# pmelchior/scarlet

Hardware: AMD Instinct MI355X
Metric: PGM iters/sec over batched blends; achieved HBM GB/s vs roofline (higher is better)
Workload: dtype f32; 1 GPU; configs[2]: 1024 independent 5-band 128x128 blends in total, 10 ExtendedSource components (41x41) each, ConvolutionRenderer FFT 160x160; iterations 0..1234 of a fit from the initial parameters; loop=blend, blends_total=1024, components_per_blend=10, sub_ranges_per_gpu=3

## Files before the change

### include/scarlet_amd.h

```cpp
#ifndef SCARLET_AMD_H
#define SCARLET_AMD_H

#include <stdint.h>

#ifdef __cplusplus
extern "C" {
#endif

typedef enum smi_status {
    SMI_OK = 0,
    SMI_ERR_INVALID = -1,
    SMI_ERR_HIP = -2,
    SMI_ERR_NO_DEVICE = -3,
    SMI_ERR_ARITHMETIC = -4
} smi_status;

const char *smi_last_error(void);
int smi_device_count(void);
const char *smi_version(void);


int smi_prox_weighted_monotonic_f32(float *flat_img, const float *weights,
                                    const int32_t *offsets, int32_t n_off,
                                    const int32_t *dist_idx, int32_t n_idx,
// ... 390 lines not shown
int smi_batch_restore_state(smi_batch *b);

int smi_batch_enable_timing(smi_batch *b, int32_t on);
int smi_batch_get_timing(smi_batch *b, double *ms_per_phase, int32_t n_phases);

int smi_batch_fft_shape(smi_batch *b, int32_t *fft_h, int32_t *fft_w);

int smi_batch_resize_test(smi_batch *b, int32_t *margin, double *edge_pull);
int smi_batch_get_component_states(smi_batch *b, const int32_t *components, int32_t n,
                                   float *states);
int smi_batch_update_components(smi_batch *b, const smi_components *c, const int32_t *keep,
                                const float *states);
int smi_batch_set_states(smi_batch *b, const int32_t *state);
int smi_batch_set_iteration_base(smi_batch *b, const int32_t *base);
int smi_batch_get_progress(smi_batch *b, int32_t *state, int32_t *n_loss);
int smi_batch_set_pause_at(smi_batch *b, const int32_t *it);
int smi_batch_get_converged(smi_batch *b, int32_t *flag);
int smi_batch_set_round(smi_batch *b, const int32_t *state, const int32_t *base,
                        const int32_t *pause_at);
int smi_batch_get_round(smi_batch *b, int32_t *state, int32_t *n_loss, int32_t *converged);

int64_t smi_observation_uploads(void);

int smi_batch_conv_path_used(smi_batch *b, int32_t *path);

int smi_batch_set_frame_extents(smi_batch *b, const int32_t *h, const int32_t *w);

int smi_fft_shape_for(int32_t H, int32_t W, int32_t kernel_h, int32_t kernel_w, int32_t conv_path,
                      int32_t *Fy, int32_t *Fx);

typedef struct smi_resampler smi_resampler;
int smi_resampler_create(const float *A, const float *Pt, int32_t C, int32_t n_a, int32_t n_b,
                         int32_t Fy, int32_t Fx, smi_resampler **out);
int smi_resampler_render(smi_resampler *r, const float *model, float *out);
int smi_resampler_time(smi_resampler *r, int32_t n_rep, double *ms_per_render);
int smi_resampler_destroy(smi_resampler *r);
int smi_resampler_get_path(smi_resampler *r, int32_t *path);
int smi_resampler_set_path(smi_resampler *r, int32_t path);

int smi_gemm_plan(int32_t M, int32_t N, int32_t K, int32_t n_batch, int64_t scratch_elems,
                  int32_t plan[5]);
int smi_gemm_test(const float *A, int64_t strideA, const float *B, int64_t strideB, float *C,
                  int64_t strideC, int32_t n_batch, int32_t M, int32_t N, int32_t K,
                  int64_t scratch_elems, int32_t plan[5], int32_t *guard_ok);
int smi_resampler_adjoint(smi_resampler *r, const float *resid, float *gpad);

int smi_sqrt_rn_normal_test(const float *x, float *y, int64_t n);

int smi_update_launch_plan_test(int32_t n_items, int32_t size_class, int64_t stage_bytes,
                                int32_t cu_count, int32_t range_items, int32_t finalize_pending,
                                int32_t n_ranges, int64_t plan[8]);
int smi_update_last_fold_plan_test(int64_t plan[8]);

int smi_batch_attach_lowres(smi_batch *b, smi_resampler *r, const int32_t *channels,
                            const float *data, const float *weights, double log_norm);
int smi_batch_get_lowres_rendered(smi_batch *b, int32_t index, float *out);


int smi_starlet_transform_f32(const float *d_images, int32_t n, int32_t H, int32_t W,
                              int32_t scales, int32_t generation, double *d_coeffs,
                              double *d_work, void *stream);
int smi_starlet_transform_f64(const double *d_images, int32_t n, int32_t H, int32_t W,
                              int32_t scales, int32_t generation, double *d_coeffs,
                              double *d_work, void *stream);
int smi_starlet_reconstruction_f64(const double *d_coeffs, int32_t n, int32_t H, int32_t W,
                                   int32_t scales, int32_t generation, double *d_image,
                                   double *d_work, void *stream);
int smi_multiresolution_support_f64(const double *d_coeffs, int32_t n, int32_t planes,
                                    int32_t H, int32_t W, int64_t plane_stride,
                                    int64_t image_stride, const double *sigma0,
                                    const double *thresh0, double K, double epsilon,
                                    int32_t max_iter, int32_t *d_support, double *d_masked,
                                    int32_t *iterations, void *stream);
int smi_coadd_f32(const float *d_images, int32_t bands, int32_t H, int32_t W, float *d_out,
                  void *stream);
int smi_coadd_f64(const double *d_images, int32_t bands, int32_t H, int32_t W, double *d_out,
                  void *stream);

typedef struct smi_detect_task {
    int32_t bands, h, w, scales;
    int64_t image_off, coeff_off, work_off;
    double sigma0, thresh0;
} smi_detect_task;
int smi_detect_wavelets_scratch_bytes(int32_t n, int64_t *bytes);
int smi_detect_wavelets_f32(int32_t n, const smi_detect_task *tasks, const void *d_tasks, double K,
                            double epsilon, int32_t max_iter, int32_t generation,
                            const float *d_images, int64_t n_images, double *d_coeffs,
                            int64_t n_coeffs, double *d_work, int64_t n_work, double *d_masked,
                            int32_t *d_support, int32_t *d_iterations, void *d_scratch,
                            int64_t scratch_bytes, void *stream);
int smi_detect_wavelets_f64(int32_t n, const smi_detect_task *tasks, const void *d_tasks, double K,
                            double epsilon, int32_t max_iter, int32_t generation,
                            const double *d_images, int64_t n_images, double *d_coeffs,
                            int64_t n_coeffs, double *d_work, int64_t n_work, double *d_masked,
                            int32_t *d_support, int32_t *d_iterations, void *d_scratch,
                            int64_t scratch_bytes, void *stream);

int smi_get_footprints_f32(const float *image, int32_t H, int32_t W, double min_separation,
                           int32_t min_area, int32_t thresh, int32_t *counts);
int smi_get_footprints_f64(const double *image, int32_t H, int32_t W, double min_separation,
                           int32_t min_area, int32_t thresh, int32_t *counts);
int smi_footprints_fetch(int32_t *bounds, uint8_t *masks, int32_t *peak_start, int32_t *peak_yx,
                         double *peak_flux);

int smi_footprints_device_work_bytes(int32_t P, int32_t H, int32_t W, int64_t *bytes);
int smi_footprints_device_fetch_bytes(const int32_t *counts, int64_t *bytes);
// ... 51 lines not shown
```

### scarlet_amd/_lib.py

```python

import ctypes
import os

import numpy as np

_HERE = os.path.dirname(os.path.abspath(__file__))
LIB_PATH = os.environ.get("SCARLET_AMD_LIB") or os.path.join(_HERE, "libscarlet_amd.so")

PROX_MONOTONIC = 1
PROX_SYMMETRY = 2
PROX_POSITIVE = 4
PROX_CENTER_ON = 8
PROX_NORM_MAX = 16
PROX_NORM_SUM = 32
PROX_L1 = 64
PROX_L0 = 128
PROX_FIT_CENTER = 256
PROX_BG_THRESH = 512
PROX_L_RELATIVE = 1024
PROX_MONO_MASK = 2048
SCHEME_AMSGRAD, SCHEME_FISTA = 0, 1
COMPONENT_POINT_SOURCE = 1 << 16
COMPONENT_SHIFTING = 1 << 17
COMPONENT_FIXED_SED = 1 << 18
# ... 124 lines not shown
        ctypes.c_int,
        [c_f64p, ctypes.c_int32, ctypes.c_int32, c_f64p, ctypes.c_int32, c_i32p, c_i32p,
         c_i32p, c_i32p, c_f64p],
    ),
    "smi_reweight_f32": (ctypes.c_int, _REWEIGHT(c_f32p)),
    "smi_reweight_f64": (ctypes.c_int, _REWEIGHT(c_f64p)),
    "smi_lite_spectra_f32": (ctypes.c_int, _LITE_SPECTRA(c_f32p)),
    "smi_lite_spectra_f64": (ctypes.c_int, _LITE_SPECTRA(c_f64p)),
    "smi_get_valid_monotonic_pixels_f32": (
        ctypes.c_int,
        [ctypes.c_int32, ctypes.c_int32, c_f32p, ctypes.c_int32, ctypes.c_int32, c_u8p, c_u8p,
         ctypes.c_double, c_i32p, ctypes.c_double],
    ),
    "smi_get_valid_monotonic_pixels_f64": (
        ctypes.c_int,
        [ctypes.c_int32, ctypes.c_int32, c_f64p, ctypes.c_int32, ctypes.c_int32, c_u8p, c_u8p,
         ctypes.c_double, c_i32p, ctypes.c_double],
    ),
    "smi_linear_interpolate_invalid_pixels_f32": (
        ctypes.c_int,
        [c_i32p, c_i32p, ctypes.c_int32, c_u8p, c_f32p, ctypes.c_int32, ctypes.c_int32, c_u8p,
         ctypes.c_double, ctypes.c_int32, c_i32p],
    ),
    "smi_linear_interpolate_invalid_pixels_f64": (
        ctypes.c_int,
        [c_i32p, c_i32p, ctypes.c_int32, c_u8p, c_f64p, ctypes.c_int32, ctypes.c_int32, c_u8p,
         ctypes.c_double, ctypes.c_int32, c_i32p],
    ),
    "smi_resampler_create": (
        ctypes.c_int,
        [c_f32p, c_f32p, ctypes.c_int32, ctypes.c_int32, ctypes.c_int32, ctypes.c_int32,
         ctypes.c_int32, ctypes.POINTER(ctypes.c_void_p)],
    ),
    "smi_resampler_render": (ctypes.c_int, [ctypes.c_void_p, c_f32p, c_f32p]),
    "smi_resampler_time": (ctypes.c_int, [ctypes.c_void_p, ctypes.c_int32,
                                          ctypes.POINTER(ctypes.c_double)]),
    "smi_resampler_destroy": (ctypes.c_int, [ctypes.c_void_p]),
    "smi_resampler_get_path": (ctypes.c_int, [ctypes.c_void_p, ctypes.POINTER(ctypes.c_int32)]),
    "smi_resampler_set_path": (ctypes.c_int, [ctypes.c_void_p, ctypes.c_int32]),
    "smi_resampler_adjoint": (ctypes.c_int, [ctypes.c_void_p, c_f32p, c_f32p]),
    "smi_gemm_plan": (ctypes.c_int, [ctypes.c_int32] * 4 + [ctypes.c_int64, c_i32p]),
    "smi_gemm_test": (
        ctypes.c_int,
        [c_f32p, ctypes.c_int64, c_f32p, ctypes.c_int64, c_f32p, ctypes.c_int64]
        + [ctypes.c_int32] * 4 + [ctypes.c_int64, c_i32p, c_i32p],
    ),
    "smi_sqrt_rn_normal_test": (ctypes.c_int, [c_f32p, c_f32p, ctypes.c_int64]),
    "smi_update_launch_plan_test": (
        ctypes.c_int,
        [ctypes.c_int32, ctypes.c_int32, ctypes.c_int64] + [ctypes.c_int32] * 4
        + [ctypes.POINTER(ctypes.c_int64)],
    ),
    "smi_update_last_fold_plan_test": (ctypes.c_int, [ctypes.POINTER(ctypes.c_int64)]),
    "smi_batch_attach_lowres": (
        ctypes.c_int, [ctypes.c_void_p, ctypes.c_void_p, c_i32p, c_f32p, c_f32p, ctypes.c_double]
    ),
    "smi_batch_get_lowres_rendered": (ctypes.c_int, [ctypes.c_void_p, ctypes.c_int32, c_f32p]),
    "smi_batch_create": (
        ctypes.c_int,
        [ctypes.POINTER(BatchDesc), ctypes.c_int, ctypes.POINTER(ctypes.c_void_p)],
    ),
    "smi_batch_destroy": (ctypes.c_int, [ctypes.c_void_p]),
    "smi_batch_add_sweep_plan": (
        ctypes.c_int,
        [ctypes.c_void_p, ctypes.c_int32, ctypes.c_int32, c_f64p, c_i32p, c_i32p,
         ctypes.c_int32],
    ),
    "smi_sweep_ring_plan": (
        ctypes.c_int,
        [ctypes.c_int32, ctypes.c_int32, c_f64p, c_i32p, c_i32p, ctypes.c_int32, c_i32p, c_f32p,
         ctypes.POINTER(ctypes.c_uint16), ctypes.c_int64],
    ),
    "smi_batch_set_observation": (ctypes.c_int, [ctypes.c_void_p, c_f32p, c_f32p]),
    "smi_batch_set_observation_device": (
        ctypes.c_int, [ctypes.c_void_p, ctypes.c_void_p, ctypes.c_void_p]
    ),
    "smi_batch_set_kernel": (ctypes.c_int, [ctypes.c_void_p, c_f32p]),
    "smi_batch_set_components": (ctypes.c_int, [ctypes.c_void_p, ctypes.POINTER(Components)]),
    "smi_batch_set_moments": (ctypes.c_int, [ctypes.c_void_p] + [c_f32p] * 6),
    "smi_batch_get_moments": (ctypes.c_int, [ctypes.c_void_p] + [c_f32p] * 6),
    "smi_batch_get_parameters": (ctypes.c_int, [ctypes.c_void_p, c_f32p, c_f32p]),
    "smi_batch_set_parameters": (ctypes.c_int, [ctypes.c_void_p, c_f32p, c_f32p]),
    "smi_batch_get_centers": (ctypes.c_int, [ctypes.c_void_p] + [c_f64p] * 5),
    "smi_batch_set_center_moments": (ctypes.c_int, [ctypes.c_void_p] + [c_f64p] * 3),
    "smi_batch_set_centers": (ctypes.c_int, [ctypes.c_void_p, c_f64p]),
    "smi_batch_get_model_morphology": (ctypes.c_int, [ctypes.c_void_p, c_f32p]),
    "smi_batch_get_starlet": (ctypes.c_int, [ctypes.c_void_p] + [c_f32p] * 5),
    "smi_batch_get_profiles": (ctypes.c_int, [ctypes.c_void_p] + [c_f64p] * 5),
    "smi_batch_set_profile_moments": (ctypes.c_int, [ctypes.c_void_p] + [c_f64p] * 3),
    "smi_profile_probe": (ctypes.c_int, [ctypes.c_int, ctypes.c_int32, c_f64p] + [ctypes.c_int32] * 4
                          + [c_f64p]),
    "smi_batch_set_starlet_moments": (ctypes.c_int, [ctypes.c_void_p] + [c_f32p] * 3),
    "smi_starlet_monotonic_mask_f32": (
        ctypes.c_int,
        [c_f32p, ctypes.c_int32, ctypes.c_int32, ctypes.c_int32, ctypes.c_int32, ctypes.c_double,
         ctypes.c_int32],
    ),
    "smi_batch_set_scheme": (ctypes.c_int, [ctypes.c_void_p, ctypes.c_int32]),
    "smi_batch_get_fista_state": (ctypes.c_int, [ctypes.c_void_p, c_f32p, c_f32p, c_f64p]),
    "smi_batch_set_fista_state": (ctypes.c_int, [ctypes.c_void_p, c_f32p, c_f32p, c_f64p]),
    "smi_batch_set_log_norm": (ctypes.c_int, [ctypes.c_void_p, ctypes.c_int32]),
    "smi_batch_add_observation": (ctypes.c_int, [ctypes.c_void_p, c_f32p, c_f32p, c_f32p]),
    "smi_batch_add_loss_constant": (ctypes.c_int, [ctypes.c_void_p, ctypes.POINTER(ctypes.c_double)]),
    "smi_batch_set_previous_loss": (ctypes.c_int, [ctypes.c_void_p, c_f64p]),
    "smi_batch_set_sub_ranges": (ctypes.c_int, [ctypes.c_void_p, ctypes.c_int32]),
    "smi_batch_get_sub_ranges": (ctypes.c_int, [ctypes.c_void_p, c_i32p]),
# ... 215 lines not shown
```

### scarlet_amd/csrc/batch.hip

```cpp
#include <rocfft/rocfft.h>

#include <algorithm>
#include <cmath>
#include <cstdlib>
#include <atomic>
#include <cstring>
#include <limits>
#include <map>
#include <mutex>
#include <thread>
#include <tuple>
#include <utility>

#include "common.h"

namespace smi {

static thread_local std::string g_error;
static std::atomic<int> g_hw_queues{4};
static std::atomic<long long> g_observation_uploads{0};
static std::mutex g_plan_mutex;
void set_error(const std::string &msg) { g_error = msg; }

static int next_fast_len(int n) {
// ... 615 lines not shown
                  int64_t scratch_elems, int32_t plan[5], int32_t *guard_ok) {
    SMI_REQUIRE(A && B && C && plan && guard_ok && scratch_elems >= 0, "bad argument");
    int ndev = 0;
    if (hipGetDeviceCount(&ndev) != hipSuccess || ndev == 0) {
        set_error("no HIP device available");
        return SMI_ERR_NO_DEVICE;
    }
    GemmPlan p;
    *guard_ok = 0;
    const int rc = gemm_test(A, strideA, B, strideB, C, strideC, n_batch, M, N, K,
                             (size_t)scratch_elems, &p, guard_ok);
    plan[0] = p.tm; plan[1] = p.tn; plan[2] = p.bk; plan[3] = p.kslice; plan[4] = p.n_slices;
    return rc;
}

int smi_sqrt_rn_normal_test(const float *x, float *y, int64_t n) {
    SMI_REQUIRE(x && y, "null argument");
    if (int rc = have_device()) return rc;
    return sqrt_rn_normal_test(x, y, n);
}

static void put_update_plan(const UpdateLaunchPlan &p, int64_t plan[8]) {
    plan[0] = p.pack;
    plan[1] = p.n_blocks;
    plan[2] = p.persistent;
    plan[3] = p.stage;
    plan[4] = (int64_t)p.lds;
    plan[5] = (int64_t)p.lds_table;
    plan[6] = p.gather_off;
    plan[7] = p.fold;
}

int smi_update_launch_plan_test(int32_t n_items, int32_t size_class, int64_t stage_bytes,
                                int32_t cu_count, int32_t range_items, int32_t finalize_pending,
                                int32_t n_ranges, int64_t plan[8]) {
    SMI_REQUIRE(plan, "null argument");
    SMI_REQUIRE(n_ranges >= 1 && n_items > 0 && range_items >= n_items && size_class >= 0 &&
                    size_class < kNumUpdateClasses && cu_count > 0 &&
                    stage_bytes < ((int64_t)1 << 31),
                "update_launch_plan_test: bad argument");
    const UpdateLaunchPlan p = update_launch_plan(n_items, size_class, stage_bytes, cu_count,
                                                  range_items, finalize_pending != 0, n_ranges > 1,
                                                  UpdateLaunchSwitches());
    put_update_plan(p, plan);
    return SMI_OK;
}

int smi_update_last_fold_plan_test(int64_t plan[8]) {
    SMI_REQUIRE(plan, "null argument");
    put_update_plan(update_last_fold_plan(), plan);
    return SMI_OK;
}

static constexpr int kMaxLowRes = 8;

int smi_batch_attach_lowres(smi_batch *b, smi_resampler *r, const int32_t *channels,
                            const float *data, const float *weights, double log_norm) {
    SMI_REQUIRE(b && r && channels && data && weights, "null argument");
    SMI_REQUIRE(b->d.n_blends == 1, "a low-resolution observation needs a batch of one blend");
    SMI_REQUIRE(!b->frame_hw, "a low-resolution observation does not support frame extents");
    SMI_REQUIRE(r->impl, "resampler already destroyed");
    SMI_REQUIRE((int)b->lowres.size() < kMaxLowRes, "too many low-resolution observations");
    SMI_HIP(hipSetDevice(b->device));
    SMI_HIP(hipStreamSynchronize(b->stream));
    if (!b->extra_terms) {
        SMI_HIP(dev_alloc(&b->extra_terms, kMaxLowRes));
        SMI_HIP(hipMemset(b->extra_terms, 0, kMaxLowRes * sizeof(double)));
    }
    LowRes *l = nullptr;
    int rc = lowres_create(r->impl, channels, data, weights, log_norm, b->d.H, b->d.W,
                           b->extra_terms + b->lowres.size(), &l);
    if (rc) {
        lowres_destroy(l);
        return rc;
    }
    b->lowres.push_back(l);
    refresh_view(b);
    return SMI_OK;
}

int smi_batch_get_lowres_rendered(smi_batch *b, int32_t index, float *out) {
    SMI_REQUIRE(b && out, "null argument");
    SMI_REQUIRE(index >= 0 && index < (int)b->lowres.size(), "no such low-resolution observation");
    return lowres_get_rendered(b->lowres[index], out, b->stream);
}

int smi_resampler_destroy(smi_resampler *r) {
    if (!r) return SMI_OK;
    resampler_destroy(r->impl);
    delete r;
    return SMI_OK;
}

int smi_get_valid_monotonic_pixels_f32(int32_t i, int32_t j, const float *image, int32_t rows,
                                       int32_t cols, uint8_t *unchecked, uint8_t *orphans,
                                       double variance, int32_t *bounds, double thresh) {
    return seam1_mask_valid<float>(i, j, image, rows, cols, unchecked, orphans, variance, bounds, thresh);
}
int smi_get_valid_monotonic_pixels_f64(int32_t i, int32_t j, const double *image, int32_t rows,
                                       int32_t cols, uint8_t *unchecked, uint8_t *orphans,
                                       double variance, int32_t *bounds, double thresh) {
    return seam1_mask_valid<double>(i, j, image, rows, cols, unchecked, orphans, variance, bounds, thresh);
}
int smi_linear_interpolate_invalid_pixels_f32(const int32_t *ri, const int32_t *ci, int32_t n,
                                              uint8_t *unchecked, float *model, int32_t rows,
                                              int32_t cols, uint8_t *orphans, double variance,
// ... 2300 lines not shown
```

### scarlet_amd/csrc/common.h

```cpp
#pragma once

#include <hip/hip_runtime.h>
#include <stdint.h>

#include <string>
#include <vector>

#include "../../include/scarlet_amd.h"

namespace smi {

void set_error(const std::string &msg);

#define SMI_HIP(expr)                                                              \
    do {                                                                           \
        hipError_t _e = (expr);                                                    \
        if (_e != hipSuccess) {                                                    \
            smi::set_error(std::string(#expr) + ": " + hipGetErrorString(_e));     \
            return SMI_ERR_HIP;                                                    \
        }                                                                          \
    } while (0)

#define SMI_REQUIRE(cond, msg)                                                     \
    do {                                                                           \
// ... 287 lines not shown
              GemmPlan *plan, int32_t *guard_ok);
struct LowRes;
int lowres_create(Resampler *r, const int32_t *channels, const float *data, const float *weights,
                  double log_norm, int H, int W, double *term_slot, LowRes **out);
void lowres_destroy(LowRes *l);
int lowres_evaluate(LowRes *l, const float *P, int Py, int Px, int backward, hipStream_t s);
void lowres_add_gradient(LowRes *l, float *Q, int Py, int Px, hipStream_t s);
int lowres_get_rendered(LowRes *l, float *out, hipStream_t s);
int launch_sweep_timing(const SweepPlanDev *d_plans, const SweepPlanDev &host_plan, int plan_id,
                        int mode, int n_rep, float one_minus_g, int waves, int groups,
                        long long *cycles, float *images, hipStream_t s);
int sqrt_rn_normal_test(const float *x, float *y, int64_t n);
enum UpdateFold : int32_t {
    kFoldNone = 0,
    kFoldTrailing = 1,
    kFoldInGrid = 2,
    kFoldSeparate = 3,
};
struct UpdateLaunchSwitches {
    int32_t forced_pack = 0, forced_blocks = 0;
    bool may_stage = true, may_persist = true;
    int32_t fold_mode = 2;
};
struct UpdateLaunchPlan {
    int32_t pack = 1;
    int32_t n_blocks = 0;
    int32_t persistent = 0;
    int32_t stage = 0;
    int32_t gather_off = -1;
    int32_t fold = kFoldNone;
    size_t lds = 0, lds_table = 0;
};
UpdateLaunchPlan update_last_fold_plan();
UpdateLaunchPlan update_launch_plan(int32_t n_items, int32_t cls, int64_t stage_bytes, int32_t cus,
                                    int32_t range_items, bool pending, bool shared,
                                    const UpdateLaunchSwitches &sw);
void launch_resize_test(const BatchView &v, int32_t *margin, double *pull, hipStream_t s);
void launch_gather_states(const BatchView &v, const int32_t *sel, const int64_t *off, int32_t n_sel,
                          float *staging, hipStream_t s);
void launch_scatter_states(const BatchView &v, const int64_t *off, const float *staging,
                           hipStream_t s);
void launch_carry_states(const int32_t *keep, const int64_t *old_moff, const int64_t *new_moff,
                         int32_t n, float *const from[4], float *const to[4], hipStream_t s);
void launch_interleave_obs(const float *data, const float *weights, float4 *dw, int64_t planes,
                           int32_t H, int32_t W, hipStream_t s);
void launch_log_norm(const float *weights, double *log_norm, int32_t nb, int64_t n,
                     hipStream_t s);
void launch_wrap_kernel(const float *kern, float *out, int32_t n_img, int32_t ph,
                        int32_t pw, int32_t Fy, int32_t Fx, float scale, hipStream_t s);
void launch_crop(const float *P, float *out, int32_t n_img, int32_t H, int32_t W,
                 int32_t Fy, int32_t Fx, hipStream_t s);
void launch_count_active(const int32_t *state, int32_t nb, int32_t *out, hipStream_t s);

bool fused_conv_supported(int Fy, int Fx);
bool fused_conv_instantiated(int Fy, int Fx);
bool fused_conv_choose(int ny, int nx, int *Fy, int *Fx);
int launch_fused_conv(const BatchView &v, int Fy, int Fx, const float *model, const float2 *Kt,
                      int k_bands, int k_per_blend, float *out, int mode, long long *dbg,
                      hipStream_t s);
int launch_fused_conv_short(const BatchView &v, int Fy, int Fx, const float *model,
                            const float2 *Kt, int k_bands, int k_per_blend, float *out, int mode,
                            long long *dbg, hipStream_t s);
int launch_stamp_spectrum(const float *d_kern, double2 *d_tmp, float2 *Kt, int n_img, int ph,
                          int pw, int Fy, int Fx, double scale, hipStream_t s);
int launch_permute_kernel_spectrum(const float2 *Khat, float2 *Kt, int n_img, int Fy, int Fx,
                                   float scale, hipStream_t s);

template <typename T>
int sweep_host_buffers(T *flat_img, int32_t n_pix, const SweepPlanHost &plan, T min_gradient);
template <typename T>
int sweep_many_host_buffers(T *images, int32_t n_img, int32_t n_pix,
                            const std::vector<SweepPlanHost> &plans, T min_gradient);
template <typename T>
int apply_filter_host_buffers(const T *image, int32_t H, int32_t W, const T *values,
                              int32_t n_taps, const int32_t *ys, const int32_t *ye,
                              const int32_t *xs, const int32_t *xe, T *result);

}
```

### scarlet_amd/csrc/fused_conv.hip

```cpp
#include <cstdlib>
#include <type_traits>

#include "common.h"
#include "fft_regs.h"

namespace smi {

using fftk::cf;
using fftk::cmul;
using fftk::cmulc;
using fftk::ld;
using fftk::st;

namespace {

#ifndef SMI_CONV_THREADS
#define SMI_CONV_THREADS 1024
#endif
constexpr int kThreads = SMI_CONV_THREADS;
constexpr int kF2 = 16;

constexpr int conv_column_stride(int fy) { return ((fy + fy / kF2 + 3) / 8) * 8 + 4; }
constexpr size_t conv_lds_bytes(int fy, int fx) {
    return sizeof(float2) * ((size_t)(fx / 2) * conv_column_stride(fy) + 2 * fy + fx) +
// ... 315 lines not shown
                xa[k2] = ld(z[k2 * C::SY]);
                xb[k2] = ld(z[k2 * C::SY + 1]);
            }
            __builtin_amdgcn_sched_barrier(0);
            if (trip == 0) mid();
            __builtin_amdgcn_sched_barrier(0);
            auto tail = [&] {
                fftk::Dft<kF2, true>::run(va);
#pragma unroll
                for (int i = 0; i < 8; ++i) {
                    z[i * C::SY] = st(va[2 * i]);
                    z[i * C::SY + 1] = st(va[2 * i + 1]);
                }
            };
            if (b.kind == 0) {
#pragma unroll
                for (int k2 = 0; k2 < 8; ++k2) {
                    va[k2] = plus(xa[k2], xb[k2]);
                    va[15 - k2] = from_partner(minus(xa[k2], xb[k2]));
                }
                tail();
            } else if (b.kind == 1) {
                va[0] = cf{xa[0].x, xb[0].x};
                va[8] = cf{xa[0].y, xb[0].y};
#pragma unroll
                for (int k2 = 1; k2 < 8; ++k2) {
                    va[k2] = plus(xa[k2], xb[k2]);
                    va[16 - k2] = minus(xa[k2], xb[k2]);
                }
                tail();
            } else {
#pragma unroll
                for (int k2 = 0; k2 < 8; ++k2) {
                    va[k2] = plus(xa[k2], xb[k2]);
                    va[15 - k2] = minus(xa[k2], xb[k2]);
                }
                tail();
            }
        }
        lds_barrier();
    }
};


template <int FX1, int NX1, int M>
struct ModelGather {
    static constexpr uint32_t kNone = 0x40000000u;
    const BatchView &v;
    int band_c, H, W, y, n2, ylo;
    struct Lanes {
        int oy, ox, h, w, mo;
        float sd;
    };
    __device__ __forceinline__ int open(unsigned long long &todo, const Lanes &l, float &sd,
                                        cf (&mv)[M]) const {
        const bool none = todo == 0;
        const int kl = none ? 0 : __builtin_ctzll(todo);
        todo &= todo - 1;
        const int oy = __builtin_amdgcn_readlane(l.oy, kl), hh = __builtin_amdgcn_readlane(l.h, kl);
        const int ox = __builtin_amdgcn_readlane(l.ox, kl), w = __builtin_amdgcn_readlane(l.w, kl);
        const float *mbase = v.morph + __builtin_amdgcn_readlane(l.mo, kl);
        const plane_t r = band_plane(mbase, hh * w);
        sd = __builtin_bit_cast(float, __builtin_amdgcn_readlane(__builtin_bit_cast(int, l.sd), kl));
        const int n1lo = (ox > 0 ? ox : 0) >> 4;
        const uint32_t hlim = none ? 0u : (uint32_t)min(hh, H - oy);
        const uint32_t wlim4 = 4u * (uint32_t)min(w, W - ox);
        const uint32_t ry = (uint32_t)(y - oy), w4 = 4u * (uint32_t)w;
        uint32_t row0, row1;
        asm("v_mul_u32_u24 %0, %1, %2" : "=v"(row0) : "v"(ry), "s"(w4));
        asm("v_mul_u32_u24 %0, %1, %2" : "=v"(row1) : "v"(ry + 1u), "s"(w4));
        row0 = ry < hlim ? row0 : kNone;
        row1 = ry + 1u < hlim ? row1 : kNone;
        const uint32_t x4 = (uint32_t)(16 * n1lo + n2 - ox) * 4u;
#pragma unroll
        for (int m = 0; m < M; ++m) {
            uint32_t t = x4 + 64u * m;
            t = t < wlim4 ? t : kNone;
            mv[m].x = __builtin_bit_cast(float, __builtin_amdgcn_raw_buffer_load_b32(r, row0 + t, 0, 0));
            mv[m].y = __builtin_bit_cast(float, __builtin_amdgcn_raw_buffer_load_b32(r, row1 + t, 0, 0));
        }
        return none ? -1 : n1lo;
    }
    __device__ __forceinline__ void close(int n1lo_, float sd_, const cf (&mv)[M], cf (&acc)[FX1]) const {
        const cf sd = cf{sd_, sd_};
        fftk::static_for<0, NX1>([&](auto lo) {
            constexpr int n1lo = decltype(lo)::value;
            if (n1lo_ == n1lo) {
#pragma unroll
                for (int m = 0; m < M; ++m)
                    if (n1lo + m < NX1) acc[n1lo + m] = fftk::fma2(mv[m], sd, acc[n1lo + m]);
                asm volatile("; n1lo = %0" ::"n"(n1lo));
            }
        });
    }
    __device__ __forceinline__ void run(int b, int lane, cf (&acc)[FX1]) const {
#pragma unroll
        for (int n1 = 0; n1 < NX1; ++n1) acc[n1] = cf{0.f, 0.f};
        const int cs = v.comp_start[b], ce = v.comp_start[b + 1];
        for (int kb = cs; kb < ce; kb += 64) {
            const int kk = kb + lane;
            const bool have = kk < ce;
            Lanes l;
            l.oy = have ? v.c_oy[kk] : 0;
            l.ox = have ? v.c_ox[kk] : 0;
            l.h = have ? v.c_h[kk] : 0;
            l.w = have ? v.c_w[kk] : 0;
            l.mo = have ? (int)v.c_moff[kk] : 0;
            l.sd = have ? v.sed[kk * v.C + band_c] : 0.f;
            const bool hit = have && l.oy < ylo + 8 && l.oy + l.h > ylo && l.oy < H && l.ox < W &&
                             l.ox + l.w > 0;
            unsigned long long todo = __ballot(hit);
            if (!todo) continue;
            cf mva[M], mvb[M];
            float sda, sdb;
            int na = open(todo, l, sda, mva);
            for (;;) {
                const int nb = open(todo, l, sdb, mvb);
                close(na, sda, mva, acc);
                if (nb < 0) break;
                na = open(todo, l, sda, mva);
                close(nb, sdb, mvb, acc);
                if (na < 0) break;
            }
        }
    }
};

extern __shared__ __attribute__((aligned(16))) float2 lds_conv[];

template <int FY1, int FX1, int ZB, bool EXT>
__global__ __launch_bounds__(kThreads) void fused_conv_kernel(BatchView v, const float *model,
                                                              const float2 *Kt, int k_bands,
                                                              int k_per_blend, float *out,
                                                              int mode, long long *dbg) {
    using C = Cfg<FY1, FX1, ZB>;
    constexpr int NX1 = C::NX1;
    const int total = gridDim.x;
    int lid = blockIdx.x;
    if (total % 8 == 0) lid = (blockIdx.x % 8) * (total / 8) + blockIdx.x / 8;
    const int b = lid / v.C + v.blend0, c = lid % v.C;
    if (v.state[b] >= 2) return;
    const int tid = threadIdx.x;
    const int H = v.H, W = v.W;
    const int Hb = EXT ? v.frame_h(b) : H, Wb = EXT ? v.frame_w(b) : W;

    Conv<FY1, FX1, ZB> cv;
    cv.T = lds_conv;
    cv.twy = cv.T + C::NT * C::SY;
    cv.twx = cv.twy + C::FY;
    cv.tid = tid;
    cv.n_pairs = (H + 1) / 2;
    cv.first_block_item();
    cv.qtab = cv.twx + C::FX;
    double *loss_part = reinterpret_cast<double *>(cv.qtab + C::FY);
    const int64_t band = ((int64_t)b * v.C + c) * H * W;
    const int n_items = cv.stride_items();
    using Item = typename Conv<FY1, FX1, ZB>::StrideItem;

    const bool have_cube = model != nullptr;
    const plane_t r_model = band_plane(have_cube ? model + band : v.data + band, H * W);
    cf mrow[FX1];
    auto fetch_model = [&](const Item &s) {
        const PairRows a = pair_rows(2 * s.j, s.n2, W);
        fftk::static_for<0, NX1>([&](auto n1c) {
            constexpr int n1 = decltype(n1c)::value;
            mrow[n1] = pair_load<n1>(r_model, a);
        });
    };
    auto render_rows = [&](const Item &s) {
        const int j0 = __builtin_amdgcn_readfirstlane(s.j - ((tid & 63) >> 4));
        if (v.render_slots <= 4) {
            const ModelGather<FX1, NX1, 4> g{v, c, Hb, Wb, 2 * s.j, s.n2, 2 * j0};
            g.run(b, tid & 63, mrow);
        } else {
            const ModelGather<FX1, NX1, (FX1 < 6 ? FX1 : 6)> g{v, c, Hb, Wb, 2 * s.j, s.n2, 2 * j0};
            g.run(b, tid & 63, mrow);
        }
    };
    if (have_cube) fetch_model(cv.stride_item(tid));
    for (int j = tid; j < C::FY; j += kThreads) {
        float s, co;
        sincospif(2.0f * (float)((j / kF2) * (j % kF2)) / (float)C::FY, &s, &co);
        cv.twy[j] = make_float2(co, -s);
    }
    for (int j = tid; j < C::FX; j += kThreads) {
        float s, co;
        sincospif(2.0f * (float)((j / kF2) * (j % kF2)) / (float)C::FX, &s, &co);
        cv.twx[j] = make_float2(co, -s);
    }
    {
        const int y0 = 2 * cv.n_pairs, tail = kF2 * C::NY1 - y0;
        for (int i = tid; i < tail * C::NT; i += kThreads)
            cv.T[(i / tail) * C::SY + sk(y0 + i % tail)] = make_float2(0.f, 0.f);
    }
    const float2 *K = Kt + ((int64_t)(k_per_blend ? b : 0) * k_bands + (k_bands == 1 ? 0 : c)) *
                               C::FY * C::NKX;
    for (int j = tid; j < C::FY; j += kThreads) cv.qtab[j] = K[(int64_t)(C::FX / 2) * C::FY + j];
    __syncthreads();
#ifndef SMI_DBG_BLOCK
#define SMI_DBG_BLOCK 0
#endif
#define SMI_STAMP(i) if (dbg && tid == 0 && blockIdx.x == SMI_DBG_BLOCK) dbg[i] = clock64()
    SMI_STAMP(0);

    for (int it = tid; (have_cube ? it : it - (tid & 63)) < n_items; it += kThreads) {
        const Item s = cv.stride_item(it);
        if (have_cube) {
            if (it != tid) fetch_model(s);
#pragma unroll
            for (int n1 = 0; n1 < NX1; ++n1)
                if (kF2 * n1 + s.n2 >= W) mrow[n1] = cf{0.f, 0.f};
        } else {
            render_rows(s);
        }
        if (s.on) cv.stride_forward(mrow, s);
    }
    lds_barrier();
    SMI_STAMP(6);
    cv.blocks_forward();
    SMI_STAMP(1);
    cv.columns(K, false);
    SMI_STAMP(2);
    double loss = 0.0;
    {
        cf loss2 = cf{0.f, 0.f};
        const int64_t pband = ((int64_t)b * v.C + c) * cv.n_pairs * W;
        const char *p_dw = reinterpret_cast<const char *>(v.dw + pband);
        const plane_t r_rendered = band_plane(out + band, H * W);
#ifndef SMI_CONV_PRE
#define SMI_CONV_PRE 8
#endif
        constexpr int kPre = SMI_CONV_PRE < NX1 ? SMI_CONV_PRE : NX1;
        cf dv[NX1], wv[NX1];
        auto fetch = [&](const Item &s, auto from, auto to) {
            uint32_t o = (uint32_t)(min(s.j, cv.n_pairs - 1) * W + s.n2) * 16u;
            asm volatile("" : "+v"(o));
            fftk::static_for<decltype(from)::value, decltype(to)::value>([&](auto n1c) {
                constexpr int n1 = decltype(n1c)::value;
                dw_load<n1>(p_dw, o, dv[n1], wv[n1]);
            });
        };
        using std::integral_constant;
        const Item s0 = cv.stride_item(tid);
        fetch(s0, integral_constant<int, 0>{}, integral_constant<int, kPre>{});
        constexpr int kLate = NX1 > 8 ? NX1 - 8 : 0;
        cv.blocks_inverse([&] { fetch(s0, integral_constant<int, kPre>{}, integral_constant<int, NX1 - kLate>{}); });
        SMI_STAMP(10);
        for (int it = tid; it < n_items; it += kThreads) {
            const Item s = cv.stride_item(it);
            const int y = 2 * s.j;
            if (it != tid) fetch(s, integral_constant<int, 0>{}, integral_constant<int, NX1 - kLate>{});
            cf m[FX1];
            cv.stride_inverse(m, s);
            fetch(s, integral_constant<int, NX1 - kLate>{}, integral_constant<int, NX1>{});
#pragma unroll
            for (int n1 = 0; n1 < NX1; ++n1) {
                const int x = kF2 * n1 + s.n2;
                if (mode == 1) {
                    plane_store(r_rendered, y, x, W, m[n1].x);
                    plane_store(r_rendered, y + 1, x, W, m[n1].y);
                }
                const cf w = x < W ? wv[n1] : cf{0.f, 0.f};
                const cf d = m[n1] - dv[n1];
                m[n1] = w * d;
// ... 55 lines not shown
    *kn = make_float2(0.5f * (a.x - b.x), 0.5f * (a.y - b.y));
}

__global__ void stamp_dft_x(const float *kern, double2 *A, int ph, int pw, int Fx, int NKX) {
    const int img = blockIdx.y;
    const int i = blockIdx.x * blockDim.x + threadIdx.x;
    if (i >= ph * NKX) return;
    const int dy = i / NKX, kx = i - dy * NKX;
    double re = 0.0, im = 0.0;
    for (int dx = 0; dx < pw; ++dx) {
        int t = (kx * (dx - pw / 2)) % Fx;
        if (t < 0) t += Fx;
        double s, c;
        sincospi(2.0 * (double)t / (double)Fx, &s, &c);
        const double k = (double)kern[((int64_t)img * ph + dy) * pw + dx];
        re += k * c;
        im -= k * s;
    }
    A[(int64_t)img * ph * NKX + i] = make_double2(re, im);
}

template <int FY1>
__global__ void stamp_dft_y(const double2 *A, float2 *Kt, int ph, int NKX, double scale) {
    constexpr int FY = FY1 * kF2;
    const int img = blockIdx.y;
    const int i = blockIdx.x * blockDim.x + threadIdx.x;
    if (i >= FY * NKX) return;
    const int ky = i / NKX, kx = i - ky * NKX;
    double re = 0.0, im = 0.0;
    for (int dy = 0; dy < ph; ++dy) {
        int t = (ky * (dy - ph / 2)) % FY;
        if (t < 0) t += FY;
        double s, c;
        sincospi(2.0 * (double)t / (double)FY, &s, &c);
        const double2 a = A[((int64_t)img * ph + dy) * NKX + kx];
        re += a.x * c + a.y * s;
        im += a.y * c - a.x * s;
    }
    Kt[((int64_t)img * NKX + column_of(kx, 2 * (NKX - 1))) * FY + pos<FY1>(ky)] =
        make_float2((float)(re * scale), (float)(im * scale));
}

#endif

template <int FY1, int FX1, int ZB, bool EXT>
int launch_ext(const BatchView &v, const float *model, const float2 *Kt, int k_bands,
               int k_per_blend, float *out, int mode, long long *dbg, hipStream_t s) {
    using C = Cfg<FY1, FX1, ZB>;
    auto kern = fused_conv_kernel<FY1, FX1, ZB, EXT>;
    static size_t configured[kMaxDevices] = {};
    if (int rc = ensure_dynamic_lds(reinterpret_cast<const void *>(kern), C::lds_bytes, configured))
        return rc;
    hipLaunchKernelGGL(kern, dim3(v.nb * v.C), dim3(kThreads), C::lds_bytes, s, v, model, Kt,
                       k_bands, k_per_blend, out, mode, dbg);
    return SMI_OK;
}

template <int FY1, int FX1, int ZB>
int launch_zb(const BatchView &v, const float *model, const float2 *Kt, int k_bands,
              int k_per_blend, float *out, int mode, long long *dbg, hipStream_t s) {
    if (v.frame_hw)
        return launch_ext<FY1, FX1, ZB, true>(v, model, Kt, k_bands, k_per_blend, out, mode, dbg, s);
    return launch_ext<FY1, FX1, ZB, false>(v, model, Kt, k_bands, k_per_blend, out, mode, dbg, s);
}

template <int FY1, int FX1>
int launch_impl(const BatchView &v, const float *model, const float2 *Kt, int k_bands,
                int k_per_blend, float *out, int mode, long long *dbg, hipStream_t s) {
    const int zy = FY1 - (v.H + kF2 - 1) / kF2, zx = FX1 - (v.W + kF2 - 1) / kF2;
    const int zb = zy < zx ? zy : zx;
    if (zb >= 2) return launch_zb<FY1, FX1, 2>(v, model, Kt, k_bands, k_per_blend, out, mode, dbg, s);
    if (zb == 1) return launch_zb<FY1, FX1, 1>(v, model, Kt, k_bands, k_per_blend, out, mode, dbg, s);
    return launch_zb<FY1, FX1, 0>(v, model, Kt, k_bands, k_per_blend, out, mode, dbg, s);
}

}

#ifndef SMI_CONV_SHORT_ROWS
bool fused_conv_supported(int Fy, int Fx) {
    auto ok = [](int f) { return f == 64 || f == 80 || f == 96 || f == 128 || f == 160; };
    if (!ok(Fy) || !ok(Fx)) return false;
    return conv_lds_bytes(Fy, Fx) <= 160 * 1024;
}

int fused_conv_length(int n) {
    for (int f : {64, 80, 96, 128, 160})
        if (f >= n) return f;
    return 0;
}

#endif

#define SMI_FUSED_DISPATCH(FN, ...)                                             \
    switch (Fy / 16 * 100 + Fx / 16) {                                          \
        case 404: return FN<4, 4>(__VA_ARGS__);                  \
        case 405: return FN<4, 5>(__VA_ARGS__);                  \
        case 406: return FN<4, 6>(__VA_ARGS__);                  \
        case 408: return FN<4, 8>(__VA_ARGS__);                  \
        case 410: return FN<4, 10>(__VA_ARGS__);                 \
        case 504: return FN<5, 4>(__VA_ARGS__);                  \
        case 505: return FN<5, 5>(__VA_ARGS__);                  \
        case 506: return FN<5, 6>(__VA_ARGS__);                  \
        case 508: return FN<5, 8>(__VA_ARGS__);                  \
        case 510: return FN<5, 10>(__VA_ARGS__);                 \
        case 604: return FN<6, 4>(__VA_ARGS__);                  \
        case 605: return FN<6, 5>(__VA_ARGS__);                  \
        case 606: return FN<6, 6>(__VA_ARGS__);                  \
        case 608: return FN<6, 8>(__VA_ARGS__);                  \
        case 610: return FN<6, 10>(__VA_ARGS__);                 \
        case 804: return FN<8, 4>(__VA_ARGS__);                  \
        case 805: return FN<8, 5>(__VA_ARGS__);                  \
        case 806: return FN<8, 6>(__VA_ARGS__);                  \
        case 808: return FN<8, 8>(__VA_ARGS__);                  \
        case 810: return FN<8, 10>(__VA_ARGS__);                 \
        case 1004: return FN<10, 4>(__VA_ARGS__);                \
        case 1005: return FN<10, 5>(__VA_ARGS__);                \
        case 1006: return FN<10, 6>(__VA_ARGS__);                \
        case 1008: return FN<10, 8>(__VA_ARGS__);                \
        case 1010: return FN<10, 10>(__VA_ARGS__);               \
        default: break;                                                         \
    }

#ifdef SMI_CONV_SHORT_ROWS
int launch_fused_conv_short(const BatchView &v, int Fy, int Fx, const float *model,
                            const float2 *Kt, int k_bands, int k_per_blend, float *out, int mode,
                            long long *dbg, hipStream_t s) {
    SMI_FUSED_DISPATCH(launch_impl, v, model, Kt, k_bands, k_per_blend, out, mode, dbg, s)
    set_error("fused convolution: FFT shape not instantiated");
    return SMI_ERR_INVALID;
}
#else
bool fused_conv_instantiated(int Fy, int Fx) { return fused_conv_supported(Fy, Fx); }

bool fused_conv_choose(int ny, int nx, int *Fy, int *Fx) {
    long best = 0;
    for (int fy : {64, 80, 96, 128, 160})
        for (int fx : {64, 80, 96, 128, 160}) {
            if (fy < ny || fx < nx || !fused_conv_supported(fy, fx)) continue;
            if (!best || (long)fy * fx < best) {
                best = (long)fy * fx;
                *Fy = fy;
// ... 60 lines not shown
```

### scarlet_amd/csrc/kernels.hip

```cpp
#include <math.h>

#include <algorithm>
#include <type_traits>
#include <stdlib.h>

#include "common.h"
#include "rounded_math.h"

namespace smi {

namespace {

constexpr int kBandChunk = 8;
constexpr int kPixBlock = 256;

template <int CTRL>
__device__ __forceinline__ float dpp_f(float v) {
    return __int_as_float(__builtin_amdgcn_update_dpp(0, __float_as_int(v), CTRL, 0xf, 0xf, false));
}
__device__ __forceinline__ float wave_sum(float v) {
    v += dpp_f<0xB1>(v);
    v += dpp_f<0x4E>(v);
    v += dpp_f<0x141>(v);
    v += dpp_f<0x140>(v);
// ... 1806 lines not shown
    }
    int bad = S.bad;
#pragma unroll
    for (int j = 0; j < NPL; ++j) {
        buf_store(r_out, slot_offset<T, LEAN>(lane, lane4, j), S.zs[j]);
        bad |= !isfinite(S.zs[j]);
    }
    if (Team<T>::any(bad) && lane == 0) atomicExch(&v.state[c.b], v.fail_code);
}

template <int NPL, int MODE, int T = 64, bool kGlobalRing = false, bool EXT = false>
__device__ __forceinline__ void update_component(const BatchView &v, const float *G, int it,
                                                 float e_rel, int prox_max_iter, int k,
                                                 float *us, float *sed_new,
                                                 const SweepPlanDev *staged = nullptr,
                                                 const char *plan_lds = nullptr, int tid = -1,
                                                 const uint32_t *gtab = nullptr) {
    constexpr bool fista = MODE == 2;
    UpdState<NPL, update_xp(T)> S;
    S.k = k;
    S.staged = staged;
    S.plan_lds = plan_lds;
    S.gtab = gtab;
    if (tid < 0) tid = (int)threadIdx.x;
    S.c = comp_ctx(v, k, T == 64 ? (tid & 63) : tid);
    if (v.state[S.c.b] >= 2) return;
    S.us = us;
    S.sed_new = sed_new;
    const float e2 = e_rel * e_rel;
    if (fista) prox_max_iter = 1;
    upd_step<NPL, MODE, T, EXT, kGlobalRing>(v, G, it, e2, prox_max_iter, S);
    team_fence<T>();
    for (int tau = 0; tau < prox_max_iter; ++tau) {
        upd_prox_begin<NPL, MODE, T>(v, S);
        team_fence<T>();
        upd_prox_plan(v, S);
        if (S.monotonic) {
            if (T == 64 || threadIdx.x < 64) {
                if (S.ring && S.ring == S.staged)
                    sweep_ring<1, (NPL > 27)>(S.us, *S.ring, S.plan_lds, S.one_minus_g, S.c.lane);
                else if (kGlobalRing && T == 64 && S.ring &&
                         __builtin_amdgcn_readfirstlane(S.ring->ring_planes) == 1)
                    sweep_ring_global<(NPL > 27)>(S.us, *S.ring, S.one_minus_g, S.c.lane);
                else
                    sweep_slots(S.us, S.slots, S.n_slots, S.one_minus_g, S.c.lane);
            }
            if (T > 64) __syncthreads();
        }
        if (upd_prox_end<NPL, MODE, T>(v, e2, S)) break;
    }
    upd_store<NPL, MODE, T>(v, S);
}

__device__ __forceinline__ int xcd_contiguous(int b, int n) {
    const int q = n >> 3, r = n & 7, x = b & 7;
    return x * q + min(x, r) + (b >> 3);
}

constexpr int update_pack_max(int npl, int team) {
    return team != 64 ? 1 : 4 * update_waves(npl, team);
}
template <int NPL, int MODE, int T, bool EXT>
__global__ __launch_bounds__(T * update_pack_max(NPL, T)) SMI_WAVES void update_kernel_reg(
    BatchView v, const float *G, int it, float e_rel, int prox_max_iter, int n_items,
    int n_finalize, int min_iter, int check, int stage_plan, int persistent, int gather_off) {
    constexpr int kPack = update_pack_max(NPL, T);
    __shared__ float sed_new[kPack][64];
    __shared__ int next_item;
    const int wave = T == 64 ? __builtin_amdgcn_readfirstlane((int)(threadIdx.x >> 6)) : 0;
    const int pack = T == 64 ? (int)(blockDim.x >> 6) : 1;
    const int n_blocks = (int)gridDim.x - n_finalize;
    if ((int)blockIdx.x >= n_blocks) {
        if (threadIdx.x < 64)
            finalize_blend(v, (int)blockIdx.x - n_blocks + v.blend0, it, e_rel, min_iter, check);
        return;
    }
    float *us = lds_dyn + wave * (T * NPL + 4) + 4;
    const SweepPlanDev *staged = nullptr;
    const char *plan_lds = nullptr;
    const uint32_t *gtab = nullptr;
    if (T == 64 && (stage_plan >= 0 || persistent)) {
        if (threadIdx.x == 0) next_item = 0;
        if (stage_plan >= 0) {
            staged = &v.plans[stage_plan];
            u32x4 *dst = reinterpret_cast<u32x4 *>(lds_dyn + pack * (T * NPL + 4));
            const u32x4 *src = static_cast<const u32x4 *>(staged->ring);
            const uint32_t n16 = staged->ring_bytes >> 4;
            for (uint32_t i = threadIdx.x; i < n16; i += blockDim.x) dst[i] = src[i];
            plan_lds = reinterpret_cast<const char *>(dst);
            if constexpr (update_gather_table(NPL, MODE, T)) {
                if (gather_off >= 0) {
                    uint32_t *tab = reinterpret_cast<uint32_t *>(lds_dyn) + (gather_off >> 2);
                    const int w = staged->w, n = staged->h * w;
                    const float inv_w = 1.0f / (float)w;
                    for (int i = threadIdx.x; i < T * NPL; i += blockDim.x) {
                        const int y = (int)(((float)i + 0.5f) * inv_w);
                        tab[i] = i < n ? (uint32_t)(y * v.Fx + (i - y * w)) * 4u : kOutOfRange;
                    }
                    gtab = tab;
                }
            }
        }
        __syncthreads();
    }
    if (T == 64 && persistent == 2 && wave == pack - 1)
        for (int bl = (int)blockIdx.x; bl < v.nb; bl += n_blocks)
            finalize_blend(v, bl + v.blend0, it, e_rel, min_iter, check);
    const bool loop = T == 64 && persistent;
    const int q = n_items / n_blocks, r = n_items % n_blocks;
    const int b = loop ? xcd_contiguous((int)blockIdx.x, n_blocks) : (int)blockIdx.x;
// ... 1036 lines not shown
```

Before: 1.501 million blend-iterations/s.

## Hoist component-metadata gather ahead of twiddle setup and generalize conv block-to-work mapping

The fused convolution kernel now loads per-component metadata (offsets, sizes, SED) for the first 64 components before the twiddle/kernel-table setup and barrier. This hides that global-memory latency behind the setup work. An optional stage (off by default, SMI_CONV_HOIST>1) also pre-opens the first model slots. Block-to-(blend, band) mapping moves into a shared conv_work_item helper with an XCD-contiguous tiled ordering, a runtime tile parameter, an env override and a test entry point. It costs extra registers for the hoisted state, which may hurt occupancy.

```diff
diff --git a/include/scarlet_amd.h b/include/scarlet_amd.h
--- a/include/scarlet_amd.h
+++ b/include/scarlet_amd.h
@@ -466,6 +466,9 @@
                                 int32_t n_ranges, int64_t plan[8]);
 int smi_update_last_fold_plan_test(int64_t plan[8]);
 
+int smi_conv_work_item_test(int32_t n_blends, int32_t n_bands, int32_t tile, int32_t *out_blend,
+                            int32_t *out_band);
+
 int smi_batch_attach_lowres(smi_batch *b, smi_resampler *r, const int32_t *channels,
                             const float *data, const float *weights, double log_norm);
 int smi_batch_get_lowres_rendered(smi_batch *b, int32_t index, float *out);
diff --git a/scarlet_amd/_lib.py b/scarlet_amd/_lib.py
--- a/scarlet_amd/_lib.py
+++ b/scarlet_amd/_lib.py
@@ -200,6 +200,7 @@
         + [ctypes.POINTER(ctypes.c_int64)],
     ),
     "smi_update_last_fold_plan_test": (ctypes.c_int, [ctypes.POINTER(ctypes.c_int64)]),
+    "smi_conv_work_item_test": (ctypes.c_int, [ctypes.c_int32] * 3 + [c_i32p, c_i32p]),
     "smi_batch_attach_lowres": (
         ctypes.c_int, [ctypes.c_void_p, ctypes.c_void_p, c_i32p, c_f32p, c_f32p, ctypes.c_double]
     ),
diff --git a/scarlet_amd/csrc/batch.hip b/scarlet_amd/csrc/batch.hip
--- a/scarlet_amd/csrc/batch.hip
+++ b/scarlet_amd/csrc/batch.hip
@@ -691,6 +691,21 @@
     return SMI_OK;
 }
 
+int smi_conv_work_item_test(int32_t n_blends, int32_t n_bands, int32_t tile, int32_t *out_blend,
+                            int32_t *out_band) {
+    SMI_REQUIRE(out_blend && out_band, "null argument");
+    SMI_REQUIRE(n_blends >= 1 && n_bands >= 1 && tile >= 0 &&
+                    (int64_t)n_blends * n_bands < ((int64_t)1 << 30) &&
+                    (int64_t)tile * n_bands < ((int64_t)1 << 30),
+                "conv_work_item_test: bad argument");
+    for (int32_t block = 0; block < n_blends * n_bands; ++block) {
+        const ConvWorkItem w = conv_work_item(block, n_blends, n_bands, tile);
+        out_blend[block] = w.blend;
+        out_band[block] = w.band;
+    }
+    return SMI_OK;
+}
+
 static constexpr int kMaxLowRes = 8;
 
 int smi_batch_attach_lowres(smi_batch *b, smi_resampler *r, const int32_t *channels,
diff --git a/scarlet_amd/csrc/common.h b/scarlet_amd/csrc/common.h
--- a/scarlet_amd/csrc/common.h
+++ b/scarlet_amd/csrc/common.h
@@ -363,7 +363,26 @@
                  int32_t Fy, int32_t Fx, hipStream_t s);
 void launch_count_active(const int32_t *state, int32_t nb, int32_t *out, hipStream_t s);
 
+__host__ __device__ __forceinline__ int xcd_contiguous(int b, int n) {
+    const int q = n >> 3, r = n & 7, x = b & 7;
+    return x * q + (x < r ? x : r) + (b >> 3);
+}
+
+struct ConvWorkItem {
+    int blend, band;
+};
+__host__ __device__ __forceinline__ ConvWorkItem conv_work_item(int block, int n_blends, int C,
+                                                                int tile) {
+    if (tile <= 0) return ConvWorkItem{block / C, block % C};
+    const int pos = xcd_contiguous(block, n_blends * C);
+    const int t = pos / (tile * C), r = pos % (tile * C);
+    const int b_lo = t * tile;
+    const int nt = tile < n_blends - b_lo ? tile : n_blends - b_lo;
+    return ConvWorkItem{b_lo + r % nt, r / nt};
+}
+
 bool fused_conv_supported(int Fy, int Fx);
+int fused_conv_tile(int grid);
 bool fused_conv_instantiated(int Fy, int Fx);
 bool fused_conv_choose(int ny, int nx, int *Fy, int *Fx);
 int launch_fused_conv(const BatchView &v, int Fy, int Fx, const float *model, const float2 *Kt,
diff --git a/scarlet_amd/csrc/fused_conv.hip b/scarlet_amd/csrc/fused_conv.hip
--- a/scarlet_amd/csrc/fused_conv.hip
+++ b/scarlet_amd/csrc/fused_conv.hip
@@ -391,8 +391,10 @@
         int oy, ox, h, w, mo;
         float sd;
     };
+    template <int N>
     __device__ __forceinline__ int open(unsigned long long &todo, const Lanes &l, float &sd,
-                                        cf (&mv)[M]) const {
+                                        cf (&mv)[N]) const {
+        static_assert(N >= M, "slots");
         const bool none = todo == 0;
         const int kl = none ? 0 : __builtin_ctzll(todo);
         todo &= todo - 1;
@@ -420,7 +422,8 @@
         }
         return none ? -1 : n1lo;
     }
-    __device__ __forceinline__ void close(int n1lo_, float sd_, const cf (&mv)[M], cf (&acc)[FX1]) const {
+    template <int N>
+    __device__ __forceinline__ void close(int n1lo_, float sd_, const cf (&mv)[N], cf (&acc)[FX1]) const {
         const cf sd = cf{sd_, sd_};
         fftk::static_for<0, NX1>([&](auto lo) {
             constexpr int n1lo = decltype(lo)::value;
@@ -432,54 +435,138 @@
             }
         });
     }
-    __device__ __forceinline__ void run(int b, int lane, cf (&acc)[FX1]) const {
-#pragma unroll
-        for (int n1 = 0; n1 < NX1; ++n1) acc[n1] = cf{0.f, 0.f};
-        const int cs = v.comp_start[b], ce = v.comp_start[b + 1];
-        for (int kb = cs; kb < ce; kb += 64) {
-            const int kk = kb + lane;
-            const bool have = kk < ce;
-            Lanes l;
-            l.oy = have ? v.c_oy[kk] : 0;
-            l.ox = have ? v.c_ox[kk] : 0;
-            l.h = have ? v.c_h[kk] : 0;
-            l.w = have ? v.c_w[kk] : 0;
-            l.mo = have ? (int)v.c_moff[kk] : 0;
-            l.sd = have ? v.sed[kk * v.C + band_c] : 0.f;
-            const bool hit = have && l.oy < ylo + 8 && l.oy + l.h > ylo && l.oy < H && l.ox < W &&
-                             l.ox + l.w > 0;
-            unsigned long long todo = __ballot(hit);
+    __device__ __forceinline__ Lanes meta(int kb, int ce, int lane) const {
+        const int kk = kb + lane;
+        const bool have = kk < ce;
+        Lanes l;
+        l.oy = have ? v.c_oy[kk] : 0;
+        l.ox = have ? v.c_ox[kk] : 0;
+        l.h = have ? v.c_h[kk] : 0;
+        l.w = have ? v.c_w[kk] : 0;
+        l.mo = have ? (int)v.c_moff[kk] : 0;
+        l.sd = have ? v.sed[kk * v.C + band_c] : 0.f;
+        return l;
+    }
+    __device__ __forceinline__ unsigned long long hits(const Lanes &l, bool have) const {
+        const bool hit = have && l.oy < ylo + 8 && l.oy + l.h > ylo && l.oy < H && l.ox < W &&
+                         l.ox + l.w > 0;
+        return __ballot(hit);
+    }
+    template <int N>
+    __device__ __forceinline__ void drain(unsigned long long todo, const Lanes &l, int na, float sda,
+                                          cf (&mva)[N], cf (&mvb)[N], cf (&acc)[FX1]) const {
+        float sdb;
+        for (;;) {
+            const int nb = open(todo, l, sdb, mvb);
+            close(na, sda, mva, acc);
+            if (nb < 0) break;
+            na = open(todo, l, sda, mva);
+            close(nb, sdb, mvb, acc);
+            if (na < 0) break;
+        }
+    }
+    __device__ __forceinline__ void chunks(int kb, int ce, int lane, cf (&acc)[FX1]) const {
+        for (; kb < ce; kb += 64) {
+            const Lanes l = meta(kb, ce, lane);
+            unsigned long long todo = hits(l, kb + lane < ce);
             if (!todo) continue;
             cf mva[M], mvb[M];
-            float sda, sdb;
-            int na = open(todo, l, sda, mva);
+            float sda;
+            const int na = open(todo, l, sda, mva);
+            drain(todo, l, na, sda, mva, mvb, acc);
+        }
+    }
+    __device__ __forceinline__ void run(int b, int lane, cf (&acc)[FX1]) const {
+#pragma unroll
+        for (int n1 = 0; n1 < NX1; ++n1) acc[n1] = cf{0.f, 0.f};
+        chunks(v.comp_start[b], v.comp_start[b + 1], lane, acc);
+    }
+
+    template <typename Start>
+    __device__ __forceinline__ void start_meta(int cs, int ce, int lane, Start &st) const {
+        st.cs = cs;
+        st.ce = ce;
+        const Lanes l = meta(cs, ce, lane);
+        st.oy = l.oy, st.ox = l.ox, st.h = l.h, st.w = l.w, st.mo = l.mo, st.sd = l.sd;
+    }
+    template <typename Start>
+    static __device__ __forceinline__ Lanes lanes_of(const Start &st) {
+        return Lanes{st.oy, st.ox, st.h, st.w, st.mo, st.sd};
+    }
+    template <typename Start>
+    __device__ __forceinline__ void start_open(int lane, Start &st) const {
+        const Lanes l = lanes_of(st);
+        st.todo = hits(l, st.cs + lane < st.ce);
+        st.na = open(st.todo, l, st.sda, st.mva);
+        st.nb = open(st.todo, l, st.sdb, st.mvb);
+    }
+    template <typename Start>
+    __device__ __forceinline__ void finish(int lane, Start &st, bool opened, cf (&acc)[FX1]) const {
+#pragma unroll
+        for (int n1 = 0; n1 < NX1; ++n1) acc[n1] = cf{0.f, 0.f};
+        const Lanes l = lanes_of(st);
+        if constexpr (M > Start::kSlots) {
+            unsigned long long todo = hits(l, st.cs + lane < st.ce);
+            if (todo) {
+                cf mva[M], mvb[M];
+                float sda;
+                const int na = open(todo, l, sda, mva);
+                drain(todo, l, na, sda, mva, mvb, acc);
+            }
+        } else {
+            if (!opened) start_open(lane, st);
+            resume(l, st, acc);
+        }
+        chunks(st.cs + 64, st.ce, lane, acc);
+    }
+    template <typename Start>
+    __device__ __forceinline__ void resume(const Lanes &l, Start &st, cf (&acc)[FX1]) const {
+        if (st.na >= 0) {
+            int na = st.na, nb = st.nb;
             for (;;) {
-                const int nb = open(todo, l, sdb, mvb);
-                close(na, sda, mva, acc);
+                close(na, st.sda, st.mva, acc);
                 if (nb < 0) break;
-                na = open(todo, l, sda, mva);
-                close(nb, sdb, mvb, acc);
+                na = open(st.todo, l, st.sda, st.mva);
+                close(nb, st.sdb, st.mvb, acc);
                 if (na < 0) break;
+                nb = open(st.todo, l, st.sdb, st.mvb);
             }
         }
     }
 };
 
+template <int MM>
+struct GatherStart {
+    static constexpr int kSlots = MM;
+    int cs, ce;
+    int oy, ox, h, w, mo;
+    float sd;
+    unsigned long long todo = 0;
+    int na = -1, nb = -1;
+    float sda, sdb;
+    cf mva[MM], mvb[MM];
+};
+
 extern __shared__ __attribute__((aligned(16))) float2 lds_conv[];
+
+#ifndef SMI_DBG_BLOCK
+#define SMI_DBG_BLOCK 0
+#endif
+#define SMI_STAMP(i) if (dbg && tid == 0 && blockIdx.x == SMI_DBG_BLOCK) dbg[i] = clock64()
 
 template <int FY1, int FX1, int ZB, bool EXT>
 __global__ __launch_bounds__(kThreads) void fused_conv_kernel(BatchView v, const float *model,
                                                               const float2 *Kt, int k_bands,
                                                               int k_per_blend, float *out,
-                                                              int mode, long long *dbg) {
+                                                              int mode, int tile, long long *dbg) {
     using C = Cfg<FY1, FX1, ZB>;
     constexpr int NX1 = C::NX1;
-    const int total = gridDim.x;
-    int lid = blockIdx.x;
-    if (total % 8 == 0) lid = (blockIdx.x % 8) * (total / 8) + blockIdx.x / 8;
-    const int b = lid / v.C + v.blend0, c = lid % v.C;
-    if (v.state[b] >= 2) return;
     const int tid = threadIdx.x;
+    SMI_STAMP(7);
+    const ConvWorkItem wi = conv_work_item(blockIdx.x, v.nb, v.C, tile);
+    const int b = wi.blend + v.blend0, c = wi.band;
+    const int state = v.state[b], comp_lo = v.comp_start[b], comp_hi = v.comp_start[b + 1];
+    if (state >= 2) return;
     const int H = v.H, W = v.W;
     const int Hb = EXT ? v.frame_h(b) : H, Wb = EXT ? v.frame_w(b) : W;
 
@@ -506,17 +593,26 @@
             mrow[n1] = pair_load<n1>(r_model, a);
         });
     };
+    constexpr int kSlotsWide = FX1 < 6 ? FX1 : 6;
+    auto with_gather = [&](const Item &s, auto &&f) {
+        const int j0 = __builtin_amdgcn_readfirstlane(s.j - ((tid & 63) >> 4));
+        if (v.render_slots <= 4)
+            f(ModelGather<FX1, NX1, 4>{v, c, Hb, Wb, 2 * s.j, s.n2, 2 * j0});
+        else
+            f(ModelGather<FX1, NX1, kSlotsWide>{v, c, Hb, Wb, 2 * s.j, s.n2, 2 * j0});
+    };
     auto render_rows = [&](const Item &s) {
-        const int j0 = __builtin_amdgcn_readfirstlane(s.j - ((tid & 63) >> 4));
-        if (v.render_slots <= 4) {
-            const ModelGather<FX1, NX1, 4> g{v, c, Hb, Wb, 2 * s.j, s.n2, 2 * j0};
-            g.run(b, tid & 63, mrow);
-        } else {
-            const ModelGather<FX1, NX1, (FX1 < 6 ? FX1 : 6)> g{v, c, Hb, Wb, 2 * s.j, s.n2, 2 * j0};
-            g.run(b, tid & 63, mrow);
-        }
+        with_gather(s, [&](const auto &g) { g.run(b, tid & 63, mrow); });
     };
+#ifndef SMI_CONV_HOIST
+#define SMI_CONV_HOIST 1
+#endif
+    GatherStart<4> gs;
+    const bool start_early = SMI_CONV_HOIST > 0 && !have_cube && tid - (tid & 63) < n_items;
+    const bool open_early = SMI_CONV_HOIST > 1 && start_early && v.render_slots <= 4;
     if (have_cube) fetch_model(cv.stride_item(tid));
+    if (start_early)
+        with_gather(cv.stride_item(tid), [&](const auto &g) { g.start_meta(comp_lo, comp_hi, tid & 63, gs); });
     for (int j = tid; j < C::FY; j += kThreads) {
         float s, co;
         sincospif(2.0f * (float)((j / kF2) * (j % kF2)) / (float)C::FY, &s, &co);
@@ -535,11 +631,13 @@
     const float2 *K = Kt + ((int64_t)(k_per_blend ? b : 0) * k_bands + (k_bands == 1 ? 0 : c)) *
                                C::FY * C::NKX;
     for (int j = tid; j < C::FY; j += kThreads) cv.qtab[j] = K[(int64_t)(C::FX / 2) * C::FY + j];
+    if (open_early) {
+        const Item s = cv.stride_item(tid);
+        const int j0 = __builtin_amdgcn_readfirstlane(s.j - ((tid & 63) >> 4));
+        const ModelGather<FX1, NX1, 4> g{v, c, Hb, Wb, 2 * s.j, s.n2, 2 * j0};
+        g.start_open(tid & 63, gs);
+    }
     __syncthreads();
-#ifndef SMI_DBG_BLOCK
-#define SMI_DBG_BLOCK 0
-#endif
-#define SMI_STAMP(i) if (dbg && tid == 0 && blockIdx.x == SMI_DBG_BLOCK) dbg[i] = clock64()
     SMI_STAMP(0);
 
     for (int it = tid; (have_cube ? it : it - (tid & 63)) < n_items; it += kThreads) {
@@ -549,6 +647,8 @@
 #pragma unroll
             for (int n1 = 0; n1 < NX1; ++n1)
                 if (kF2 * n1 + s.n2 >= W) mrow[n1] = cf{0.f, 0.f};
+        } else if (start_early && it == tid) {
+            with_gather(s, [&](const auto &g) { g.finish(tid & 63, gs, open_early, mrow); });
         } else {
             render_rows(s);
         }
@@ -710,7 +810,7 @@
     if (int rc = ensure_dynamic_lds(reinterpret_cast<const void *>(kern), C::lds_bytes, configured))
         return rc;
     hipLaunchKernelGGL(kern, dim3(v.nb * v.C), dim3(kThreads), C::lds_bytes, s, v, model, Kt,
-                       k_bands, k_per_blend, out, mode, dbg);
+                       k_bands, k_per_blend, out, mode, fused_conv_tile(v.nb * v.C), dbg);
     return SMI_OK;
 }
 
@@ -745,6 +845,16 @@
     for (int f : {64, 80, 96, 128, 160})
         if (f >= n) return f;
     return 0;
+}
+
+int fused_conv_tile(int grid) {
+    static const int forced = [] {
+        const char *e = getenv("SMI_CONV_TILE");
+        const int t = e ? atoi(e) : -1;
+        return t <= 4096 ? t : -1;
+    }();
+    if (forced >= 0) return forced;
+    return grid % 8 == 0 ? 1 : 0;
 }
 
 #endif
diff --git a/scarlet_amd/csrc/kernels.hip b/scarlet_amd/csrc/kernels.hip
--- a/scarlet_amd/csrc/kernels.hip
+++ b/scarlet_amd/csrc/kernels.hip
@@ -1882,10 +1882,6 @@
     upd_store<NPL, MODE, T>(v, S);
 }
 
-__device__ __forceinline__ int xcd_contiguous(int b, int n) {
-    const int q = n >> 3, r = n & 7, x = b & 7;
-    return x * q + min(x, r) + (b >> 3);
-}
 
 constexpr int update_pack_max(int npl, int team) {
     return team != 64 ? 1 : 4 * update_waves(npl, team);
```

Result: slower. 1.478 million blend-iterations/s (-1.6%).
